# wallisc/TracerBoy

Measured on AMD Instinct MI355X. Metric: Msamples/s (WxHxspp/s), higher is better.
Workload: dtype f32; 1 GPU; cornell-box 1920x1080 64spp depth8; triangles=36, bvh_builder=sah, pipeline=lockstep, parallelism=tiles1, scene_in_lds=True, kernel_variant=matte

## Files before the change

include/tracerboy_hip.h:

```cpp
#ifndef TRACERBOY_HIP_H
#define TRACERBOY_HIP_H

#include <stdint.h>
#include "tb_abi.h"

#ifdef __cplusplus
extern "C" {
#endif

#define TB_OK 0
#define TB_E_INVALID -1
#define TB_E_NO_DEVICE -2
#define TB_E_IO -3
#define TB_E_PARSE -4
#define TB_E_DEVICE -5
#define TB_E_UNSUPPORTED -6
#define TB_E_NO_SCENE -7

typedef struct tb_context tb_context;

typedef struct tb_camera {
    float Position[3], LookAt[3], Right[3], Up[3];
    float LensHeight, FocalDistance;
} tb_camera;
// ... 135 lines not shown
typedef struct tb_launch_plan {
    int32_t pipeline;
    uint32_t groups;
    uint32_t high_occupancy_copy, full_variant;
    uint32_t stack_lds_entries, stack_overflow_entries;
    uint32_t compact_nodes;
    uint32_t prepass;
    uint32_t overlap_launches;
    uint32_t batch_frames, frame_group;
    uint32_t rule_pipeline, rule_copy, rule_prepass;
    uint32_t guided_groups;
    uint32_t costly_first;
} tb_launch_plan;
void tb_plan_defaults(tb_plan_input* in);
int tb_variant_waves_hi(const char* variant_name);
int tb_variant_stash_entries(const char* variant_name);
int tb_plan_launch(const tb_plan_input* in, tb_launch_plan* out);
uint32_t tb_frame_groups(uint32_t frames, uint32_t frame_group, uint32_t guided, uint32_t group, uint32_t* first_frame, uint32_t* num_frames);

int tb_host_scene_view(tb_context* ctx, TbSceneView* view);
int tb_make_frame_constants(tb_context* ctx, uint32_t width, uint32_t height, uint32_t frame,
                            const tb_output_settings* settings, float time_seed, TbPerFrameConstants* out);
float tb_last_render_ms(tb_context* ctx);
int tb_trace_closest(tb_context* ctx, uint32_t n, const float* origins, const float* dirs, float* out_t,
                     int32_t* out_material, float* out_bary, uint32_t* out_prim, uint32_t* out_geom,
                     float* out_normal, float* out_uv, uint32_t* out_boxes, uint32_t* out_tris);
int tb_device_math(tb_context* ctx, int fn, uint32_t n, const float* a, const float* b, float* out);

typedef struct tb_host_scene tb_host_scene;
int tb_host_scene_load(const char* pbrt_path, int bvh_builder, int load_flags, tb_host_scene** out, char* err, uint32_t err_len);
// ... 16 lines not shown
```

tracerboy_amd/api.py:

```python
import ctypes as C
import os

import numpy as np

from . import _ctypes_abi as abi

_HERE = os.path.dirname(os.path.abspath(__file__))
LIB_PATH = os.environ.get("TB_LIB", os.path.join(_HERE, "libtracerboy_hip.so"))

_lib = None


class TracerBoyError(RuntimeError):
    def __init__(self, code, message):
        super().__init__("tracerboy_hip error %d: %s" % (code, message))
        self.code = code


def lib():
    global _lib
    if _lib is not None:
        return _lib
    if not os.path.exists(LIB_PATH):
        raise ImportError("libtracerboy_hip.so is not built: run `python -m tracerboy_amd.build` "
# ... 29 lines not shown
        "tb_render_realtime": (C.c_int, [vp, C.c_uint32, C.c_uint32, P(abi.tb_output_settings), P(abi.tb_denoiser_settings), C.c_float]),
        "tb_read_realtime": (C.c_int, [vp, C.c_int, vp]),
        "tb_post_process": (C.c_int, [vp, P(abi.tb_post_settings), C.c_uint32, vp, vp]),
        "tb_read_averaged_luminance": (C.c_int, [vp, P(C.c_float)]),
        "tb_write_image_rgba8": (C.c_int, [C.c_char_p, C.c_uint32, C.c_uint32, vp]),
        "tb_write_image_f32": (C.c_int, [C.c_char_p, C.c_uint32, C.c_uint32, vp]),
        "tb_decode_image": (C.c_int, [C.c_char_p, P(C.c_uint32), P(C.c_uint32), P(C.c_int), P(C.c_int), vp]),
        "tb_read_aov": (C.c_int, [vp, C.c_int, vp]),
        "tb_accum_device_ptr": (C.c_int, [vp, P(vp), P(vp)]),
        "tb_read_stats": (C.c_int, [vp, P(abi.tb_readback_stats)]),
        "tb_read_wave_profile": (C.c_int, [vp, P(C.c_uint64)]),
        "tb_read_split_profile": (C.c_int, [vp, P(C.c_uint64)]),
        "tb_plan_defaults": (None, [P(abi.tb_plan_input)]),
        "tb_plan_launch": (C.c_int, [P(abi.tb_plan_input), P(abi.tb_launch_plan)]),
        "tb_variant_waves_hi": (C.c_int, [C.c_char_p]),
        "tb_invalidate_history": (None, [vp]),
        "tb_samples_rendered": (C.c_uint32, [vp]),
        "tb_select_pixel": (C.c_int, [vp, C.c_uint32, C.c_uint32]),
        "tb_set_tile_assignment": (C.c_int, [vp, C.c_uint32, C.c_uint32, C.c_uint32, C.c_uint32]),
        "tb_owned_pixels": (C.c_uint64, [vp, C.c_uint32, C.c_uint32]),
        "tb_pack_owned_device": (C.c_int, [vp, vp]),
        "tb_pack_owned_device_async": (C.c_int, [vp, vp]),
        "tb_stream": (vp, [vp]),
        "tb_unpack_gathered_device": (C.c_int, [vp, vp, vp, C.c_uint64, C.c_uint32, C.c_uint32, C.c_uint32, C.c_uint32, C.c_uint32, vp]),
        "tb_unpack_gathered_host": (C.c_int, [C.c_uint32, C.c_uint32, C.c_uint32, C.c_uint32, C.c_uint32, P(vp), vp]),
        "tb_set_option": (C.c_int, [vp, C.c_char_p, C.c_int64]),
        "tb_get_option": (C.c_int64, [vp, C.c_char_p]),
        "tb_host_scene_view": (C.c_int, [vp, P(abi.TbSceneView)]),
        "tb_make_frame_constants": (C.c_int, [vp, C.c_uint32, C.c_uint32, C.c_uint32, P(abi.tb_output_settings), C.c_float, P(abi.TbPerFrameConstants)]),
        "tb_last_render_ms": (C.c_float, [vp]),
# ... 31 lines not shown
    s = abi.tb_denoiser_settings()
    lib().tb_default_denoiser_settings(C.byref(s))
    return s


def GetDefaultPostProcessSettings():
    s = abi.tb_post_settings()
    lib().tb_default_post_settings(C.byref(s))
    return s


def VariantWavesHi(name):
    return int(lib().tb_variant_waves_hi(name.encode()))


def VariantStashEntries(name):
    return int(lib().tb_variant_stash_entries(name.encode()))


def PlanLaunch(**kw):
    pin = abi.tb_plan_input(); lib().tb_plan_defaults(C.byref(pin))
    for k, v in kw.items():
        if not hasattr(pin, k): raise KeyError(k)
        setattr(pin, k, v)
    plan = abi.tb_launch_plan()
    rc = lib().tb_plan_launch(C.byref(pin), C.byref(plan))
    if rc != 0: raise TracerBoyError(rc, "tb_plan_launch")
    return plan


# ... 306 lines not shown
```

tracerboy_amd/build.py:

```python
import concurrent.futures as cf
import hashlib
import os
import subprocess
import sys

ROOT = os.path.dirname(os.path.abspath(__file__))
REPO = os.path.dirname(ROOT)
CSRC = os.path.join(ROOT, "csrc")
OBJ = os.path.join(ROOT, "_build")
LIB = os.path.join(ROOT, "libtracerboy_hip.so")
CLI = os.path.join(ROOT, "tracerboy-hip")
HIPCC = os.environ.get("HIPCC", "/opt/rocm/bin/hipcc")
ARCH = os.environ.get("TB_ARCH", "gfx950")

COMMON = ["-O3", "-std=c++17", "-fPIC", "-ffp-contract=off", "-fno-fast-math", "-Wall", "-Wno-unused-function",
          "-Wno-unused-variable", "-Wno-unused-but-set-variable", "-I" + os.path.join(REPO, "include")] + os.environ.get("TB_EXTRA_FLAGS", "").split()
DEVICE = ["--offload-arch=" + ARCH, "-fno-slp-vectorize", "-mllvm", "-amdgpu-sched-strategy=max-ilp"]
SCHED_MEMORY_CLAUSE = ["-mllvm", "-amdgpu-sched-strategy=max-memory-clause"]
TU_SCHEDULER = {"kernels/pt_variant_vol4.hip": SCHED_MEMORY_CLAUSE, "kernels/pt_variant_surf.hip": SCHED_MEMORY_CLAUSE}


def device_flags(src):
    if src not in TU_SCHEDULER:
        return DEVICE
    base = [f for i, f in enumerate(DEVICE) if not f.startswith("-amdgpu-sched-strategy=")
            and not (f == "-mllvm" and i + 1 < len(DEVICE) and DEVICE[i + 1].startswith("-amdgpu-sched-strategy="))]
    return base + TU_SCHEDULER[src]

HOST_SRCS = ["host/pbrt_loader.cpp", "host/pbf_loader.cpp", "host/host_scene.cpp", "host/images.cpp", "host/image_decode.cpp", "host/image_formats.cpp", "host/bvh_build.cpp", "host/procedural.cpp", "host/context.cpp", "host/context_scene.cpp", "host/context_render.cpp", "host/pbrt_dump.cpp"]
KERNEL_SRCS = ["kernels/pt_kernels.hip", "kernels/post_kernels.hip", "kernels/bvh_kernels.hip", "kernels/rt_kernels.hip", "kernels/pt_variant_matte.hip", "kernels/pt_variant_matte5.hip", "kernels/pt_variant_env.hip", "kernels/pt_variant_env5.hip", "kernels/pt_variant_surf.hip",
               "kernels/pt_variant_sss.hip", "kernels/pt_variant_sss4.hip",
               "kernels/pt_variant_vol.hip", "kernels/pt_variant_vol4.hip", "kernels/pt_variant_full.hip",
               "kernels/pt_split_matte.hip", "kernels/pt_split_env.hip", "kernels/pt_split_surf.hip", "kernels/pt_split_sss.hip"]


def _deps_digest():
    h = hashlib.sha1()
    for base in (CSRC, os.path.join(REPO, "include")):
        for dp, _, fs in sorted(os.walk(base)):
            for f in sorted(fs):
                if f.endswith((".h", ".hpp", ".inc", ".cpp", ".hip")):
                    with open(os.path.join(dp, f), "rb") as fh:
                        h.update(f.encode()); h.update(fh.read())
    h.update(" ".join([f for f in COMMON + DEVICE if not f.startswith("-I")] + [k + " ".join(v) for k, v in sorted(TU_SCHEDULER.items())]).encode())
    return h.hexdigest()
# ... 55 lines not shown
```

tracerboy_amd/csrc/host/context.cpp:

```cpp
#include "context_internal.h"

using namespace tbhost;
using namespace tbctx;

namespace tbctx {

std::string g_createError;
std::atomic<int64_t> g_liveDeviceBytes{0};
#ifndef __HIP_DEVICE_COMPILE__
const Variant kVariants[] = {
    {0u, pt_launch_persistent_matte, "matte", pt_launch_persistent_matte5, TB_MATTE_WAVES, 0, wf_launch_matte, true, pt_launch_split_matte, 0u},
        {PT_FEAT_ENV, pt_launch_persistent_env, "env", pt_launch_persistent_env5, TB_ENV_WAVES, 1, wf_launch_env, true, pt_launch_split_env, TB_ENV_STASH},
    {PT_FEAT_ENV | PT_FEAT_SPECULAR | PT_FEAT_TEXTURES, pt_launch_persistent_surf, "surf", nullptr, 0, 2, wf_launch_surf, true, pt_launch_split_surf, 0u},
        {PT_FEAT_ENV | PT_FEAT_SPECULAR | PT_FEAT_TEXTURES | PT_FEAT_SSS, pt_launch_persistent_sss, "sss", pt_launch_persistent_sss4, TB_SSS_WAVES, 5,
            wf_launch_sss, false, pt_launch_split_sss, TB_SSS_STASH},
    {PT_FEAT_ENV | PT_FEAT_SPECULAR | PT_FEAT_TEXTURES | PT_FEAT_SSS | PT_FEAT_MIX, pt_launch_persistent_vol, "vol", pt_launch_persistent_vol4, TB_VOL_WAVES,
        3, wf_launch_vol, false, nullptr, TB_VOL_STASH},
        {PT_FEAT_ALL, pt_launch_persistent_full, "full", nullptr, 0, 4, nullptr, false, nullptr, 0u},
};
const int kNumVariants = (int)(sizeof(kVariants) / sizeof(kVariants[0]));
#endif

int fail(tb_context* c, int code, const std::string& msg) { if (c) c->err = msg; else g_createError = msg; return code; }

void ensure(DevBuf& b, size_t bytes)
{
// ... 176 lines not shown
}

int tb_material_count(tb_context* c) { return (c && c->hasScene) ? (int)c->scene.materials.size() : 0; }
int tb_get_material(tb_context* c, int id, TbMaterial* o)
{
    if (!c || !o) return TB_E_INVALID;
    if (!c->hasScene || id < 0 || id >= (int)c->scene.materials.size()) return fail(c, TB_E_INVALID, "material id out of range");
    *o = c->scene.materials[(size_t)id]; return TB_OK;
}
int tb_set_material(tb_context* c, int id, const TbMaterial* in)
{
    return guarded(c, [&]() {
        if (!in || !c->hasScene || id < 0 || id >= (int)c->scene.materials.size()) return fail(c, TB_E_INVALID, "material id out of range");
        c->scene.materials[(size_t)id] = *in;
        HIP_TRY(hipMemcpy((void*)&c->ds.materials[id].m, in, sizeof *in, hipMemcpyHostToDevice));
        if (c->sceneInLds) HIP_TRY(hipMemcpy((void*)(c->ds.ldsBlob + c->ds.offMaterials + sizeof(TbDevMaterial) * (size_t)id), in, sizeof *in,
            hipMemcpyHostToDevice));
        c->sceneFeatures = sceneFeatureMask(c->scene);
        c->ds.textureUse = sceneTextureUse(c);
        c->samplesRendered = 0;
        for (tb_context* p : c->peers) { const int rc = tb_set_material(p, id, in); if (rc != TB_OK) return rc; }
        return TB_OK;
    });
}

static int renderGroup(tb_context* c, uint32_t W, uint32_t H, uint32_t n, const tb_output_settings* s, float t)
{
    const uint32_t world = 1u + (uint32_t)c->peers.size();
    if (c->options.count("aov") && c->options["aov"]) return fail(c, TB_E_UNSUPPORTED, "tb_render: AOV targets are not gathered across the devices of a group");
    std::vector<tb_context*> all; all.push_back(c); for (tb_context* p : c->peers) all.push_back(p);
    for (uint32_t i = 0; i < world; i++) if (all[i]->tiles.world != world || all[i]->tiles.rank != i) { all[i]->tiles = TbTileMap{i, world, 64, 64};
        all[i]->samplesRendered = 0; }
// ... 285 lines not shown
    in->split_trav = 4; in->guided_groups = 1;
}
int tb_variant_stash_entries(const char* name)
{
    if (!name) return -1;
    for (int i = 0; i < tbctx::kNumVariants; i++) if (!strcmp(tbctx::kVariants[i].name, name)) return tbctx::kVariants[i].fnHi ? (int)tbctx::kVariants[i].stashHi : 0;
    return -1;
}
int tb_variant_waves_hi(const char* name)
{
    if (!name) return -1;
    for (int i = 0; i < tbctx::kNumVariants; i++) if (!strcmp(tbctx::kVariants[i].name,
        name)) return tbctx::kVariants[i].fnHi ? (int)tbctx::kVariants[i].wavesHi : 0;
    return -1;
}
uint32_t tb_frame_groups(uint32_t frames, uint32_t frameGroup, uint32_t guided, uint32_t group, uint32_t* firstFrame, uint32_t* numFrames)
{
    uint32_t lg = 0; while ((2u << lg) <= frameGroup) lg++;
    const uint32_t total = tb_fg_groups(frames, lg, guided ? 1u : 0u, 0xffffffffu, nullptr, nullptr);
    if (group < total) { uint32_t f0 = 0, l = 0; (void)tb_fg_groups(frames, lg, guided ? 1u : 0u, group, &f0, &l);
        if (firstFrame) *firstFrame = f0; if (numFrames) *numFrames = std::min(1u << l, frames - std::min(frames, f0)); }
    return total;
}

int tb_plan_launch(const tb_plan_input* in, tb_launch_plan* out)
{
    if (!in || !out || !in->width || !in->height) return TB_E_INVALID;
    PlanLaunch(*in, *out);
    return TB_OK;
}
// ... 111 lines not shown
    if (!strcmp(name, "overlap_trial_us_overlapped")) return (int64_t)(c->overlapTrial.best[0] * 1000.0f);
    if (!strcmp(name, "overlap_trial_us_one_at_a_time")) return (int64_t)(c->overlapTrial.best[1] * 1000.0f);
    if (!strcmp(name, "overlap_trial_phase")) return c->overlapTrial.phase;
    if (!strcmp(name, "last_plan_rule_pipeline")) return c->lastPlan.rule_pipeline;
    if (!strcmp(name, "last_plan_rule_copy")) return c->lastPlan.rule_copy;
    if (!strcmp(name, "last_plan_rule_prepass")) return c->lastPlan.rule_prepass;
    if (!strcmp(name, "last_plan_frame_group")) return c->lastPlan.frame_group;
    if (!strcmp(name, "last_plan_guided_groups")) return c->lastPlan.guided_groups;
    if (!strcmp(name, "last_plan_costly_first")) return c->lastPlan.costly_first;
    if (!strcmp(name, "debug_region_order_ptr")) return (int64_t)(uintptr_t)c->regionOrder[c->lastFgPar].p;
    if (!strcmp(name, "debug_region_cost_ptr")) return (int64_t)(uintptr_t)c->regionCost.p;
    if (!strcmp(name, "debug_live_device_bytes")) return g_liveDeviceBytes.load();
    if (!strcmp(name, "last_plan_stack_overflow")) return c->lastPlan.stack_overflow_entries;
    if (!strcmp(name, "last_split_waves")) return c->lastSplitWaves;
    if (!strcmp(name, "last_pipeline")) return c->lastPipeline;
    if (!strcmp(name, "last_variant")) { for (int i = 0; i < kNumVariants; i++) if (c->lastVariant == kVariants[i].name) return kVariants[i].id; return -1; }
    auto it = c->options.find(name); return it == c->options.end() ? 0 : it->second;
}

static void fillView(const HostScene& s, TbSceneView* v);
int tb_host_scene_view(tb_context* c, TbSceneView* v)
{
    if (!c || !v) return TB_E_INVALID;
    if (!c->hasScene) return fail(c, TB_E_NO_SCENE, "no scene loaded");
    fillView(c->scene, v);
    return TB_OK;
}

int tb_make_frame_constants(tb_context* c, uint32_t, uint32_t, uint32_t frame, const tb_output_settings* settings, float t, TbPerFrameConstants* out)
{
// ... 162 lines not shown
```

tracerboy_amd/csrc/host/context_internal.h:

```cpp
#pragma once
#include "host_scene.h"
#include "../kernels/pt_launch.h"
#include "../kernels/pt_device_features.h"
#include "launch_plan.h"

#include <hip/hip_runtime.h>

#include <algorithm>
#include <atomic>
#include <cstring>
#include <limits>
#include <cmath>
#include <map>
#include <stdexcept>
#include <string>
#include <vector>

using namespace tbhost;

extern "C" {
typedef hipError_t (*pt_variant_fn)(hipStream_t, const TbDeviceScene*, const TbPerFrameConstants*, const TbDeviceTargets*, uint32_t, uint32_t, uint32_t,
    uint32_t,
                                    const TbTileMap*, int, int, int);
hipError_t pt_launch_persistent_matte(hipStream_t, const TbDeviceScene*, const TbPerFrameConstants*, const TbDeviceTargets*, uint32_t, uint32_t, uint32_t,
    uint32_t, const TbTileMap*, int, int, int);
hipError_t pt_launch_persistent_env(hipStream_t, const TbDeviceScene*, const TbPerFrameConstants*, const TbDeviceTargets*, uint32_t, uint32_t, uint32_t,
    uint32_t, const TbTileMap*, int, int, int);
hipError_t pt_launch_persistent_surf(hipStream_t, const TbDeviceScene*, const TbPerFrameConstants*, const TbDeviceTargets*, uint32_t, uint32_t, uint32_t,
    uint32_t, const TbTileMap*, int, int, int);
hipError_t pt_launch_persistent_matte5(hipStream_t, const TbDeviceScene*, const TbPerFrameConstants*, const TbDeviceTargets*, uint32_t, uint32_t, uint32_t,
    uint32_t, const TbTileMap*, int, int, int);
hipError_t pt_launch_persistent_env5(hipStream_t, const TbDeviceScene*, const TbPerFrameConstants*, const TbDeviceTargets*, uint32_t, uint32_t, uint32_t,
    uint32_t, const TbTileMap*, int, int, int);
hipError_t pt_launch_persistent_sss(hipStream_t, const TbDeviceScene*, const TbPerFrameConstants*, const TbDeviceTargets*, uint32_t, uint32_t, uint32_t,
    uint32_t, const TbTileMap*, int, int, int);
hipError_t pt_launch_persistent_sss4(hipStream_t, const TbDeviceScene*, const TbPerFrameConstants*, const TbDeviceTargets*, uint32_t, uint32_t, uint32_t,
    uint32_t, const TbTileMap*, int, int, int);
hipError_t pt_launch_persistent_vol4(hipStream_t, const TbDeviceScene*, const TbPerFrameConstants*, const TbDeviceTargets*, uint32_t, uint32_t, uint32_t,
    uint32_t, const TbTileMap*, int, int, int);
hipError_t pt_launch_persistent_vol(hipStream_t, const TbDeviceScene*, const TbPerFrameConstants*, const TbDeviceTargets*, uint32_t, uint32_t, uint32_t,
    uint32_t, const TbTileMap*, int, int, int);
hipError_t pt_launch_persistent_full(hipStream_t, const TbDeviceScene*, const TbPerFrameConstants*, const TbDeviceTargets*, uint32_t, uint32_t, uint32_t,
    uint32_t, const TbTileMap*, int, int, int);
typedef hipError_t (*pt_split_fn)(hipStream_t, const TbDeviceScene*, const TbPerFrameConstants*, const TbDeviceTargets*, const TbSplitParams*, uint32_t,
    uint32_t, uint32_t, uint32_t,
// ... 20 lines not shown
hipError_t wf_launch_surf(hipStream_t, int, const TbDeviceScene*, const TbPerFrameConstants*, const WfParams*, const WfQueue*, const WfQueue*, const WfQueue*,
    const WfHits*, int, TbFloat4*, TbFloat4*, uint32_t);
hipError_t wf_launch_sss(hipStream_t, int, const TbDeviceScene*, const TbPerFrameConstants*, const WfParams*, const WfQueue*, const WfQueue*, const WfQueue*,
    const WfHits*, int, TbFloat4*, TbFloat4*, uint32_t);
hipError_t wf_launch_vol(hipStream_t, int, const TbDeviceScene*, const TbPerFrameConstants*, const WfParams*, const WfQueue*, const WfQueue*, const WfQueue*,
    const WfHits*, int, TbFloat4*, TbFloat4*, uint32_t);
}

namespace tbctx {
using namespace tbhost;

extern std::string g_createError;
#ifndef TB_MATTE_WAVES
#define TB_MATTE_WAVES 5
#endif
#ifndef TB_ENV_WAVES
#define TB_ENV_WAVES 6
#endif
#ifndef TB_SSS_WAVES
#define TB_SSS_WAVES 6
#endif
#ifndef TB_VOL_WAVES
#define TB_VOL_WAVES 4
#endif
#ifndef TB_ENV_STASH
#define TB_ENV_STASH 7
#endif
#ifndef TB_VOL_STASH
#define TB_VOL_STASH 0
#endif
#ifndef TB_SSS_STASH
#define TB_SSS_STASH 0
#endif
struct Variant { uint32_t features; pt_variant_fn fn; const char* name; pt_variant_fn fnHi; uint32_t wavesHi; int id; wf_variant_fn wf; bool pooled;
    pt_split_fn split; uint32_t stashHi; };
extern const Variant kVariants[];
extern const int kNumVariants;

extern std::atomic<int64_t> g_liveDeviceBytes;
struct DevBuf {
    void* p = nullptr; size_t bytes = 0;
    void release() { if (p) { (void)hipFree(p); g_liveDeviceBytes -= (int64_t)bytes; } p = nullptr; bytes = 0; }
};

}
using tbctx::DevBuf;

struct tb_context {
    int device = 0;
    hipStream_t stream = nullptr;
// ... 21 lines not shown
    DevBuf postOut, postRgba8, postHistogram, postAverage;
    DevBuf rtIndirect[2], rtMoment[2], rtFinal[2], rtDenoise[2], rtComposited;
    uint32_t rtActive = 0, rtWidth = 0, rtHeight = 0; int rtLast[5] = {-1, -1, -1, -1, -1};
    bool lastRenderRealtime = false; tb_camera prevCamera{};
    DevBuf wfCols[2][6], wfShadowCols[12], wfHitA, wfHitG, wfSamples, wfCounts, workCounter;
    uint64_t wfCapacity = 0, wfSampleCapacity = 0;
    int lastPipeline = 0;
    uint32_t samplesRendered = 0;
    tb_output_settings lastSettings{}; bool haveLastSettings = false;
    float lastTime = 0.0f;
    uint32_t selX = 0xffffffffu, selY = 0xffffffffu;
    TbTileMap tiles{0, 1, 64, 64};
    std::map<std::string, int64_t> options;
    float lastMs = 0.0f;
    std::string lastVariant;
    int lastNodeLayout = 0;
    int lastSlotLogCap = 0;
    struct PrepassTrial { uint64_t key = 0; int calls = 0, pending = 0, nWith = 0, nWithout = 0; float msWith = 0, msWithout = 0; bool keep = false;
        uint64_t stamp = 0; } prepassTrial;
    struct OverlapTrial { uint64_t key = 0; int phase = 0 ; int n[2] = {0, 0};
        float best[2] = {0, 0}; bool keep = true; } overlapTrial;
    struct CallRec { uint64_t key = 0; int mode = -1; bool deviceBound = false, settled = false, used = true; } callRec[8];
    hipEvent_t evCallEnd[8] = {nullptr, nullptr, nullptr, nullptr, nullptr, nullptr, nullptr, nullptr}; uint64_t callCount = 0; int lastOverlap = 0;
    tb_launch_plan lastPlan{};
    uint64_t kernelEventStamp = 0;
    uint32_t sceneGeneration = 0;
    float interiorWalkTriangleShare = 0;
    uint32_t hitPrimBits = 32, hitGeomBits = 32;
    int lastCompactHits = 0;
    DevBuf debugCounters;
// ... 64 lines not shown
```

tracerboy_amd/csrc/host/context_render.cpp:

```cpp
#include "context_internal.h"
#include "tb_vec.h"

namespace tbctx {

bool historyRelevantChange(const tb_output_settings& a, const tb_output_settings& b)
{
    return a.OutputType != b.OutputType || a.EnableNormalMaps != b.EnableNormalMaps || a.RenderModeRealTime != b.RenderModeRealTime ||
           a.DOFFocalDistance != b.DOFFocalDistance || a.ApertureWidth != b.ApertureWidth || a.FilterType != b.FilterType || a.FilterWidth != b.FilterWidth ||
           a.FireflyClampValue != b.FireflyClampValue || a.EnableNextEventEstimation != b.EnableNextEventEstimation ||
           a.EnableSamplingImportanceResampling != b.EnableSamplingImportanceResampling || a.EnableBlueNoise != b.EnableBlueNoise ||
               a.MaxBounces != b.MaxBounces ||
           a.DebugValue != b.DebugValue || a.DebugValue2 != b.DebugValue2;
}

void renderWavefront(tb_context* c, int variant, uint32_t W, uint32_t H, uint32_t firstFrame, uint32_t n, TbPerFrameConstants pf)
{
    auto opt = [&](const char* k, int64_t d) { auto it = c->options.find(k); return it == c->options.end() ? d : it->second; };
    const uint64_t pixels = (uint64_t)W * H;
    const uint64_t perFrame = (uint64_t)((W + 7) / 8) * ((H + 7) / 8) * 64;
    const uint64_t budget = (uint64_t)opt("wavefront_paths", 16ll << 20);
    const uint32_t segCap = (uint32_t)std::max<int64_t>(256, opt("wavefront_segment", 4096));
    uint32_t batch = (uint32_t)std::max<uint64_t>(1, std::min<uint64_t>(n, budget / perFrame));
    const uint64_t maxSegments = (perFrame * batch + segCap - 1) / segCap;
    const uint64_t capacity = maxSegments * segCap;
// ... 295 lines not shown
        pin.pipeline = 0; PlanLaunch(pin, plan); plan.rule_pipeline = TB_PLAN_RULE_SPLIT_NO_ROOM;
    }
    const bool wavefront = plan.pipeline == 2, pooled = plan.pipeline == 3, split = plan.pipeline == 4, groups = plan.groups != 0;
    const int64_t fg = opt("frame_group", 0);
    pt_variant_fn launch = plan.high_occupancy_copy ? v->fnHi : v->fn;
    size_t overflowHalf = 0;
    TbDeviceScene dsLaunch = c->ds; dsLaunch.stackOverflow = nullptr; dsLaunch.stackOverflowLanes = 0;
    if (plan.stack_overflow_entries) {
        const int numCUs = deviceCUs(c);
        const uint32_t lanes = 2u * 8u * (uint32_t)numCUs * 256u;
        ensure(c->stackOverflow, (size_t)plan.stack_overflow_entries * lanes * 4 * 2);
        overflowHalf = (size_t)plan.stack_overflow_entries * lanes;
        dsLaunch.stackDepth = plan.stack_lds_entries; dsLaunch.stackOverflow = (uint32_t*)c->stackOverflow.p; dsLaunch.stackOverflowLanes = lanes;
    }
    if (plan.full_variant && v != &kVariants[kNumVariants - 1]) { v = &kVariants[kNumVariants - 1]; launch = v->fn; c->lastVariant = v->name; }
    if (opt("node_layout", 0) == 1 && !twoLevel && !c->sceneInLds && !c->ds.nodesC && !c->compactTried) {
        ensureCompactNodes(c); dsLaunch.nodesC = c->ds.nodesC; dsLaunch.quant = c->ds.quant;
        pin.has_compact_nodes = c->ds.nodesC ? 1u : 0u; PlanLaunch(pin, plan);
    }
    const bool compactNodes = plan.compact_nodes != 0;
    if (!compactNodes) dsLaunch.nodesC = nullptr;
    c->lastNodeLayout = compactNodes ? 1 : 0;
    bool prepass = plan.prepass == TB_PLAN_PREPASS_ON;
    if (plan.prepass == TB_PLAN_PREPASS_TRIAL) {
        tb_context::PrepassTrial& t = c->prepassTrial;
        const uint64_t key = ((uint64_t)W << 48) ^ ((uint64_t)H << 32) ^ ((uint64_t)n << 12) ^ ((uint64_t)s.MaxBounces << 4) ^ ((uint64_t)c->sceneGeneration <<
            24) ^ (uint64_t)(uintptr_t)launch;
        if (t.key != key) { t = tb_context::PrepassTrial(); t.key = key; }
        if (t.pending) {
            float ms = 0;
// ... 90 lines not shown
                    HIP_TRY(hipMemsetAsync(c->fgSamples[par].p, 0, pixels * batch * 16, overlap ? c->side[par] : c->stream));
                }
            auto warmFrameGroupForm = [&](uint32_t par, bool withHits) {
                TbDeviceTargets warm = tg; warm.samples = (TbFloat4*)c->fgSamples[par].p; warm.workCounter = (uint32_t*)c->workCounter.p + par * 128u;
                const int numCUs = deviceCUs(c);
                if (c->fgSlotLog[par].bytes < 16ull * numCUs * 16 * 8) ensure(c->fgSlotLog[par], 16ull * numCUs * 16 * 8);
                warm.slotLog = (unsigned long long*)c->fgSlotLog[par].p; warm.slotLogCap = 16; warm.launchEpoch = ++c->launchEpoch;
                warm.primaryHits = withHits ? (unsigned long long*)c->fgHits[par].p : nullptr; warm.firstBounce = withHits && firstBounce ? 1u : 0u;
                warm.hitStamp = withHits ? hitStampOf(warm.launchEpoch) : 0u; warm.hitPrimBits = hitPrimBits; warm.hitGeomBits = c->hitGeomBits;
                TbDeviceScene dsPar = dsLaunch; if (dsPar.stackOverflow) dsPar.stackOverflow += par * overflowHalf;
                hipStream_t st = overlap ? c->side[par] : c->stream;
                HIP_TRY(launch(st, &dsPar, &pf, &warm, W, H, c->samplesRendered, 0, &c->tiles, withHits ? 0 : (c->sceneInLds ? 1 : 0), 0, 0));
                HIP_TRY(hipStreamSynchronize(st));
            };
            if (overlap && std::find(c->warmedLaunchers.begin(), c->warmedLaunchers.end(), (const void*)launch) == c->warmedLaunchers.end()) {
                if (twoLevel) { for (uint32_t par = 0; par < 2; par++) warmFrameGroupForm(par, false); }
                else {
                    TbDeviceTargets none = tg; none.samples = nullptr;
                    TbDeviceScene dsWarm = c->ds; dsWarm.nodesC = nullptr;
                    for (uint32_t par = 0; par < 2; par++)
                        HIP_TRY(launch(c->side[par], &dsWarm, &pf, &none, W, H, c->samplesRendered, 0, &c->tiles, c->sceneInLds ? 1 : 0, 0, 0));
                }
                c->warmedLaunchers.push_back((const void*)launch);
            }
            if (prepass) {
                for (uint32_t par = 0; par < 2u; par++)
                    if (c->fgHits[par].bytes < pixels * batch * hitRecordBytes) {
                        HIP_TRY(hipStreamSynchronize(c->side[par])); HIP_TRY(hipStreamSynchronize(c->stream));
                        ensure(c->fgHits[par], pixels * batch * hitRecordBytes);
                        HIP_TRY(hipMemsetAsync(c->fgHits[par].p, 0, pixels * batch * hitRecordBytes, overlap ? c->side[par] : c->stream));
                    }
// ... 61 lines not shown
```

tracerboy_amd/csrc/host/context_scene.cpp:

```cpp
#include "context_internal.h"

namespace tbctx {

void releaseScene(tb_context* c)
{
    for (DevBuf& b : c->sceneBufs) b.release();
    c->sceneBufs.clear();
    memset(&c->ds, 0, sizeof c->ds);
}

uint32_t sceneFeatureMask(const HostScene& s)
{
    uint32_t f = 0;
    if (!s.envMap.empty()) f |= PT_FEAT_ENV;
    for (const TbMaterial& m : s.materials) {
        if ((m.Flags & TB_MAT_NO_SPECULAR) == 0 && (m.Flags & TB_MAT_MIX) == 0) f |= PT_FEAT_SPECULAR;
        if (m.albedoIndex != TB_INVALID_TEXTURE || m.emissiveIndex != TB_INVALID_TEXTURE || m.specularMapIndex != TB_INVALID_TEXTURE ||
            m.normalMapIndex != TB_INVALID_TEXTURE) f |= PT_FEAT_TEXTURES | PT_FEAT_SPECULAR;
        if (m.Flags & TB_MAT_SUBSURFACE_SCATTER) f |= PT_FEAT_SSS;
        if (m.Flags & TB_MAT_MIX) f |= PT_FEAT_MIX;
    }
    for (const TbLight& l : s.lights) if (l.LightType != TB_LIGHT_TYPE_AREA) f |= PT_FEAT_EXT;
    return f;
}
// ... 306 lines not shown
        }
        {
            std::vector<TbTriB> perm(s.trisB.size() * TB_LDS_TRI_COPIES);
            for (size_t i = 0; i < s.trisB.size(); i++)
                for (int kz = 0; kz < 3; kz++)
                    for (int sw = 0; sw < 2; sw++) {
                        int kx = kz == 2 ? 0 : kz + 1, ky = kx == 2 ? 0 : kx + 1;
                        if (sw) std::swap(kx, ky);
                        const TbTriB& t = s.trisB[i]; TbTriB q = t;
                        const float* src[3] = {t.v0, t.v1, t.v2}; float* dst[3] = {q.v0, q.v1, q.v2};
                        for (int v = 0; v < 3; v++) { dst[v][0] = src[v][kx]; dst[v][1] = src[v][ky]; dst[v][2] = src[v][kz]; }
                        perm[i * TB_LDS_TRI_COPIES + (size_t)(kz * 2 + sw)] = q;
                    }
            d.offTris = put(perm.data(), perm.size() * sizeof(TbTriB));
        }
        d.offHitGroups = put(devHit.data(), devHit.size() * sizeof(TbDevHitGroup));
        d.offIndices = put(s.indexBuffer.data(), s.indexBuffer.size() * 4);
        d.offVertices = put(s.vertexBuffer.data(), s.vertexBuffer.size() * 4);
        d.offMaterials = put(devMat.data(), devMat.size() * sizeof(TbDevMaterial));
        d.offLights = put(devLight.data(), devLight.size() * sizeof(TbDevLight));
        while (blob.size() % 16) blob.push_back(0);
        size_t budget = (size_t)opt("lds_scene_budget", 40 * 1024);
        c->sceneInLds = blob.size() + (size_t)d.stackDepth * 256 * 4 <= budget && opt("scene_in_lds", 1) != 0 && !twoLevel;
        if (c->sceneInLds) { d.ldsBlob = upload(c, blob); d.ldsBlobBytes = (uint32_t)blob.size(); }
        else { d.ldsBlob = nullptr; d.ldsBlobBytes = 0; }
        d.parkMin = (uint32_t)std::max<int64_t>(1, opt("park_min", c->sceneInLds ? 2 : 24));
    }
    HIP_TRY(hipStreamSynchronize(c->stream));
    c->sceneFeatures = sceneFeatureMask(s);
    c->hasScene = true;
    c->samplesRendered = 0;
}

}
```

tracerboy_amd/csrc/host/launch_plan.h:

```cpp
#pragma once
#include <stdint.h>
#include <algorithm>
#include "../../../include/tracerboy_hip.h"
#include "../kernels/pt_scene.h"

namespace tbhost {

inline void PlanLaunch(const tb_plan_input& in, tb_launch_plan& p)
{
    p = tb_launch_plan{};
    const bool plain = !in.count_rays && !in.aov && !in.realtime && !in.selected_pixel;
    const int64_t pipe = in.pipeline == 4 ? 0 : in.pipeline;
    p.pipeline = (int32_t)pipe;
    if (in.pipeline == 4 && in.variant_has_split && plain && !in.two_level) {
        const uint64_t trav = (uint64_t)std::max<int64_t>(1, in.split_trav),
            shade = in.split_shade > 0 ? (uint64_t)in.split_shade : (in.scene_in_lds ? 4u : 6u);
        uint64_t ring = 256; while (ring < 256u * shade) ring *= 2;
        const uint64_t entries = (in.split_stack_cap > 0 && (uint64_t)in.split_stack_cap < in.stack_depth && !in.scene_in_lds) ? (uint64_t)in.split_stack_cap :
            in.stack_depth;
        const uint64_t lds = entries * trav * 256u + (in.scene_in_lds ? ((uint64_t)in.lds_blob_bytes + 15u) / 16u * 16u : 0u) + shade * 128u * 48u + ring *
            4u + 16u;
        const bool fits = lds <= 160u * 1024u && 4ull * std::max<uint64_t>(1, in.owned_regions) <= 0xfffffull && (trav + shade) * 64u <= 1024u;
        if (fits) { p.pipeline = 4; p.rule_pipeline = TB_PLAN_RULE_SPLIT; return; }
        p.rule_pipeline = TB_PLAN_RULE_SPLIT_NO_ROOM;
// ... 72 lines not shown
```

tracerboy_amd/csrc/kernels/pt_common.hpp:

```cpp
#pragma once
#include <hip/hip_runtime.h>
#include "pt_device.hpp"

namespace {
using namespace pt;

constexpr int BLOCK = 256;

template <bool SCENE_LDS>
__device__ __forceinline__ void make_refs(SceneRefs& sc, const TbDeviceScene& ds, const uint8_t* blob)
{
    if (SCENE_LDS) {
        sc.nodes = blob + ds.offNodes; sc.tris = (const TbTriB*)__builtin_assume_aligned(blob + ds.offTris, 16); sc.trisPermuted = 1;
        sc.hitGroups = (const TbDevHitGroup*)(blob + ds.offHitGroups); sc.indices = (const uint32_t*)(blob + ds.offIndices);
        sc.vertices = (const float*)(blob + ds.offVertices); sc.materials = (const TbDevMaterial*)(blob + ds.offMaterials);
        sc.lights = (const TbDevLight*)(blob + ds.offLights);
    } else {
        sc.nodes = (const uint8_t*)ds.nodes; sc.tris = ds.tris; sc.trisPermuted = 0; sc.hitGroups = ds.hitGroups; sc.indices = ds.indexBuffer;
            sc.vertices = ds.vertexBuffer;
        sc.materials = ds.materials; sc.lights = ds.lights;
    }
    sc.numHitGroups = ds.numHitGroups; sc.numIndices = ds.numIndices; sc.numVertexFloats = ds.numVertexFloats;
    sc.numMaterials = ds.numMaterials; sc.numLights = ds.numLights;
}

__device__ __forceinline__ bool block_region(const TbTileMap& tiles, uint32_t W, uint32_t H, uint32_t region, uint32_t& bx, uint32_t& by)
{
    if (tiles.world <= 1) { const uint32_t blocksX = (W + 15u) / 16u; bx = region % blocksX; by = region / blocksX; return true; }
    const uint32_t subX = tiles.tileW / 16u, perTile = subX * (tiles.tileH / 16u);
    const uint32_t k = region / perTile, sub = region % perTile;
    const uint32_t tilesX = (W + tiles.tileW - 1) / tiles.tileW, t = tiles.rank + k * tiles.world;
    bx = (t % tilesX) * subX + sub % subX; by = (t / tilesX) * (tiles.tileH / 16u) + sub / subX;
    return true;
}

__device__ __noinline__ uint32_t claim_work_item(uint32_t* counters, uint32_t regions, uint32_t numGroups, uint32_t banded, const uint32_t* order = nullptr)
// ... 67 lines not shown
```

tracerboy_amd/csrc/kernels/pt_scene.h:

```cpp
#pragma once
#include "../../../include/tb_abi.h"
#include <stdint.h>

#define TB_LDS_NODE_STRIDE 80u
#define TB_DEVICE_REF_MASK 0x7fffffffu
#define TB_LDS_TRI_COPIES 6u

struct __attribute__((aligned(16))) TbDevHitGroup { uint32_t MaterialIndex, vFirst, iFirst, pad; };
struct __attribute__((aligned(16))) TbDevMaterial { TbMaterial m; uint32_t pad[3]; };
struct __attribute__((aligned(16))) TbDevLight { TbLight l; uint32_t pad[2]; };

struct TbDeviceScene {
    const TbNodeB* nodes;
    const TbTriB* tris;
    const TbNodeC* nodesC;
    TbQuantFrame quant;
    uint32_t rootRef;
    const TbInstanceB* instances; uint32_t numInstances;
    uint32_t numNodes, numTris;
    float rootCenter[3], rootHalf[3];
    const TbDevHitGroup* hitGroups;      uint32_t numHitGroups;
    const uint32_t* indexBuffer;         uint32_t numIndices;
    const float* vertexBuffer;           uint32_t numVertexFloats;
    const TbDevMaterial* materials;      uint32_t numMaterials;
    const TbTextureData* textureData;    uint32_t numTextureData;
    const TbDevLight* lights;            uint32_t numLights;
    const TbImageDesc* images;           uint32_t numImages;
    const TbFloat4* texelPool;
    const TbFloat4* envMap;              uint32_t envWidth, envHeight;
    const TbFloat4* blueNoise0;
    const TbFloat4* blueNoise1;
    TbConfigConstants config;
    uint32_t alphaTest;
    uint32_t textureUse;
    uint32_t parkMin;
    uint32_t stackDepth;
    uint32_t* stackOverflow;     uint32_t stackOverflowLanes;
    const uint8_t* ldsBlob;      uint32_t ldsBlobBytes;
    uint32_t offNodes, offTris, offHitGroups, offIndices, offVertices, offMaterials, offLights;
};

#ifndef TB_COSTLY_STEP
#define TB_COSTLY_STEP 8
#endif
struct TbDeviceTargets {
    TbFloat4* output;
    TbFloat4* jittered;
    TbFloat4* aovNormals;
    TbFloat4* aovWorldPos0, *aovWorldPos1;
    TbFloat4* aovCustom;
    float* aovDepth;
    TbFloat4* aovEmissive;
    uint32_t* stats;
    unsigned long long* rayStats;
// ... 66 lines not shown
```

tracerboy_amd/csrc/kernels/pt_variant.inc:

```
#include <hip/hip_runtime.h>
#include "pt_common.hpp"
#include "pt_launch.h"

namespace {
#include "pt_persistent.inc"
#ifndef PT_ONLY_PERSISTENT
#include "pt_stream.inc"
#endif
}

#define PT_CAT2(a, b) a##b
#define PT_CAT(a, b) PT_CAT2(a, b)

extern "C" hipError_t PT_CAT(pt_launch_persistent_, PT_NAME)(hipStream_t stream, const TbDeviceScene* ds, const TbPerFrameConstants* pf,
    const TbDeviceTargets* tg,
                                                            uint32_t W, uint32_t H, uint32_t firstFrame, uint32_t numFrames, const TbTileMap* tiles,
                                                            int sceneInLds, int countRays, int pipeline)
{
    uint32_t blocks = tb_persistent_grid(W, H, *tiles);
    if (blocks == 0) return hipSuccess;
    size_t lds = (size_t)ds->stackDepth * BLOCK * 4 + (sceneInLds ? ds->ldsBlobBytes : 0);
#ifdef PT_LDS_STASH
    if (!sceneInLds && tg->samples && !ds->numInstances) lds += (size_t)PT_LDS_STASH * BLOCK * 4;
#endif
// ... 15 lines not shown
            uint32_t lgG = 0; while ((2u << lgG) <= tg->frameGroup) lgG++; \
            const uint64_t items = (uint64_t)blocks * tb_fg_groups(numFrames, lgG, guidedLaunch ? 1u : 0u, 0xffffffffu, nullptr, nullptr), \
                resident = (uint64_t)(perCU > 0 ? perCU : 1) * numCUs; \
            grid.x = (uint32_t)(items < 2 * resident ? items : 2 * resident);  \
            if (grid.x == 0) grid.x = 1;  \
            if (!tg->slotLog || !tg->slotLogCap || grid.x > 16u * (uint32_t)numCUs) return hipErrorInvalidValue; \
            e = hipMemsetAsync(tg->slotLog, 0, (size_t)grid.x * tg->slotLogCap * 8, stream); if (e != hipSuccess) return e; \
            e = hipMemsetAsync(tg->workCounter, 0, 512, stream); if (e != hipSuccess) return e; } \
        hipLaunchKernelGGL((__VA_ARGS__), grid, block, lds, stream, *ds, *pf, *tg, W, H, firstFrame, numFrames, *tiles); } while (0)
#ifndef PT_ONLY_PERSISTENT
#define PT_PICK(L, C) do { if (pipeline == 1) PT_LAUNCH(pt_stream<PT_FEATURES, L, C>); else PT_LAUNCH(pt_persistent<PT_FEATURES, L, C, false>); } while (0)
#else
#define PT_PICK(L, C) do { if (pipeline != 0) return hipErrorInvalidValue; PT_LAUNCH(pt_persistent<PT_FEATURES, L, C, false>); } while (0)
#endif
    if (tg->samples && (countRays || pipeline != 0)) return hipErrorInvalidValue;
#if PT_COUNT
    if (countRays) { if (sceneInLds) PT_PICK(true, true); else PT_PICK(false, true); return hipGetLastError(); }
#else
    if (countRays) return hipErrorInvalidValue;
#endif
#ifdef PT_ONLY_PERSISTENT
    if (ds->numInstances) {
        if (!tg->samples || sceneInLds || ds->nodesC) return hipErrorInvalidValue;
        if (ds->stackOverflow) {
            if (ds->stackOverflowLanes < 2u * 8u * (uint32_t)numCUs * BLOCK) return hipErrorInvalidValue;
            PT_LAUNCH(pt_persistent<PT_FEATURES, false, false, true, true, false, true>);
        } else PT_LAUNCH(pt_persistent<PT_FEATURES, false, false, true, false, false, true>);
        return hipGetLastError();
    }
#elif !(PT_FEATURES & PT_FEAT_EXT)
// ... 61 lines not shown
        if (ds->stackOverflowLanes < 2u * 8u * (uint32_t)numCUs * BLOCK) return hipErrorInvalidValue;
        if (sceneInLds) PT_LAUNCH(pt_persistent<PT_FEATURES, true, false, true, true>); else PT_LAUNCH(pt_persistent<PT_FEATURES, false, false, true, true>);
        return hipGetLastError();
    }
#endif
    if (ds->stackOverflow) return hipErrorInvalidValue;
#ifdef TB_EXP_PROFILE_GROUPS
    if (tg->samples) { if (sceneInLds) PT_LAUNCH(pt_persistent<PT_FEATURES, true, true, true>);
        else PT_LAUNCH(pt_persistent<PT_FEATURES, false, true, true>); }
#else
    if (tg->samples) { if (guidedLaunch) PT_LAUNCH(pt_persistent<PT_FEATURES, true, false, true, false, false, false, false, false, true>);
        else if (sceneInLds) PT_LAUNCH(pt_persistent<PT_FEATURES, true, false, true>);
        else PT_LAUNCH(pt_persistent<PT_FEATURES, false, false, true>); }
#endif
    else if (sceneInLds) PT_PICK(true, false); else PT_PICK(false, false);
#undef PT_PICK
#undef PT_LAUNCH
    return hipGetLastError();
}

#if !(PT_FEATURES & PT_FEAT_EXT) && !defined(PT_ONLY_PERSISTENT)
#include "wf_types.h"
#define PT_HAS_POOLED (!(PT_FEATURES & (PT_FEAT_SSS | PT_FEAT_MIX)))
namespace {
#include "wf_kernels.inc"
#if PT_HAS_POOLED
#include "pt_pooled.inc"
#endif
}
extern "C" hipError_t PT_CAT(wf_launch_, PT_NAME)(hipStream_t stream, int stage, const TbDeviceScene* ds, const TbPerFrameConstants* pf, const WfParams* wp,
// ... 65 lines not shown
```

Measured before the change: 7170 Msamples/s.

## Keep only BVH in LDS and add a six-wave matte LDS kernel copy

```diff
diff --git a/include/tracerboy_hip.h b/include/tracerboy_hip.h
--- a/include/tracerboy_hip.h
+++ b/include/tracerboy_hip.h
@@ -173,6 +173,7 @@
 } tb_launch_plan;
 void tb_plan_defaults(tb_plan_input* in);
 int tb_variant_waves_hi(const char* variant_name);
+int tb_variant_waves_lds(const char* variant_name);
 int tb_variant_stash_entries(const char* variant_name);
 int tb_plan_launch(const tb_plan_input* in, tb_launch_plan* out);
 uint32_t tb_frame_groups(uint32_t frames, uint32_t frame_group, uint32_t guided, uint32_t group, uint32_t* first_frame, uint32_t* num_frames);
diff --git a/tracerboy_amd/api.py b/tracerboy_amd/api.py
--- a/tracerboy_amd/api.py
+++ b/tracerboy_amd/api.py
@@ -67,6 +67,7 @@
         "tb_plan_defaults": (None, [P(abi.tb_plan_input)]),
         "tb_plan_launch": (C.c_int, [P(abi.tb_plan_input), P(abi.tb_launch_plan)]),
         "tb_variant_waves_hi": (C.c_int, [C.c_char_p]),
+        "tb_variant_waves_lds": (C.c_int, [C.c_char_p]),
         "tb_invalidate_history": (None, [vp]),
         "tb_samples_rendered": (C.c_uint32, [vp]),
         "tb_select_pixel": (C.c_int, [vp, C.c_uint32, C.c_uint32]),
@@ -128,6 +129,10 @@
     return int(lib().tb_variant_waves_hi(name.encode()))
 
 
+def VariantWavesLds(name):
+    return int(lib().tb_variant_waves_lds(name.encode()))
+
+
 def VariantStashEntries(name):
     return int(lib().tb_variant_stash_entries(name.encode()))
 
diff --git a/tracerboy_amd/build.py b/tracerboy_amd/build.py
--- a/tracerboy_amd/build.py
+++ b/tracerboy_amd/build.py
@@ -17,7 +17,8 @@
           "-Wno-unused-variable", "-Wno-unused-but-set-variable", "-I" + os.path.join(REPO, "include")] + os.environ.get("TB_EXTRA_FLAGS", "").split()
 DEVICE = ["--offload-arch=" + ARCH, "-fno-slp-vectorize", "-mllvm", "-amdgpu-sched-strategy=max-ilp"]
 SCHED_MEMORY_CLAUSE = ["-mllvm", "-amdgpu-sched-strategy=max-memory-clause"]
-TU_SCHEDULER = {"kernels/pt_variant_vol4.hip": SCHED_MEMORY_CLAUSE, "kernels/pt_variant_surf.hip": SCHED_MEMORY_CLAUSE}
+SCHED_DEFAULT = []
+TU_SCHEDULER = {"kernels/pt_variant_vol4.hip": SCHED_MEMORY_CLAUSE, "kernels/pt_variant_surf.hip": SCHED_MEMORY_CLAUSE, "kernels/pt_variant_matte6.hip": SCHED_DEFAULT}
 
 
 def device_flags(src):
@@ -28,7 +29,7 @@
     return base + TU_SCHEDULER[src]
 
 HOST_SRCS = ["host/pbrt_loader.cpp", "host/pbf_loader.cpp", "host/host_scene.cpp", "host/images.cpp", "host/image_decode.cpp", "host/image_formats.cpp", "host/bvh_build.cpp", "host/procedural.cpp", "host/context.cpp", "host/context_scene.cpp", "host/context_render.cpp", "host/pbrt_dump.cpp"]
-KERNEL_SRCS = ["kernels/pt_kernels.hip", "kernels/post_kernels.hip", "kernels/bvh_kernels.hip", "kernels/rt_kernels.hip", "kernels/pt_variant_matte.hip", "kernels/pt_variant_matte5.hip", "kernels/pt_variant_env.hip", "kernels/pt_variant_env5.hip", "kernels/pt_variant_surf.hip",
+KERNEL_SRCS = ["kernels/pt_kernels.hip", "kernels/post_kernels.hip", "kernels/bvh_kernels.hip", "kernels/rt_kernels.hip", "kernels/pt_variant_matte.hip", "kernels/pt_variant_matte5.hip", "kernels/pt_variant_matte6.hip", "kernels/pt_variant_env.hip", "kernels/pt_variant_env5.hip", "kernels/pt_variant_surf.hip",
                "kernels/pt_variant_sss.hip", "kernels/pt_variant_sss4.hip",
                "kernels/pt_variant_vol.hip", "kernels/pt_variant_vol4.hip", "kernels/pt_variant_full.hip",
                "kernels/pt_split_matte.hip", "kernels/pt_split_env.hip", "kernels/pt_split_surf.hip", "kernels/pt_split_sss.hip"]
diff --git a/tracerboy_amd/csrc/host/context.cpp b/tracerboy_amd/csrc/host/context.cpp
--- a/tracerboy_amd/csrc/host/context.cpp
+++ b/tracerboy_amd/csrc/host/context.cpp
@@ -9,7 +9,8 @@
 std::atomic<int64_t> g_liveDeviceBytes{0};
 #ifndef __HIP_DEVICE_COMPILE__
 const Variant kVariants[] = {
-    {0u, pt_launch_persistent_matte, "matte", pt_launch_persistent_matte5, TB_MATTE_WAVES, 0, wf_launch_matte, true, pt_launch_split_matte, 0u},
+    {0u, pt_launch_persistent_matte, "matte", pt_launch_persistent_matte5, TB_MATTE_WAVES, 0, wf_launch_matte, true, pt_launch_split_matte, 0u,
+        pt_launch_persistent_matte6, TB_MATTE_LDS_WAVES},
         {PT_FEAT_ENV, pt_launch_persistent_env, "env", pt_launch_persistent_env5, TB_ENV_WAVES, 1, wf_launch_env, true, pt_launch_split_env, TB_ENV_STASH},
     {PT_FEAT_ENV | PT_FEAT_SPECULAR | PT_FEAT_TEXTURES, pt_launch_persistent_surf, "surf", nullptr, 0, 2, wf_launch_surf, true, pt_launch_split_surf, 0u},
         {PT_FEAT_ENV | PT_FEAT_SPECULAR | PT_FEAT_TEXTURES | PT_FEAT_SSS, pt_launch_persistent_sss, "sss", pt_launch_persistent_sss4, TB_SSS_WAVES, 5,
@@ -216,8 +217,6 @@
         if (!in || !c->hasScene || id < 0 || id >= (int)c->scene.materials.size()) return fail(c, TB_E_INVALID, "material id out of range");
         c->scene.materials[(size_t)id] = *in;
         HIP_TRY(hipMemcpy((void*)&c->ds.materials[id].m, in, sizeof *in, hipMemcpyHostToDevice));
-        if (c->sceneInLds) HIP_TRY(hipMemcpy((void*)(c->ds.ldsBlob + c->ds.offMaterials + sizeof(TbDevMaterial) * (size_t)id), in, sizeof *in,
-            hipMemcpyHostToDevice));
         c->sceneFeatures = sceneFeatureMask(c->scene);
         c->ds.textureUse = sceneTextureUse(c);
         c->samplesRendered = 0;
@@ -533,6 +532,12 @@
         name)) return tbctx::kVariants[i].fnHi ? (int)tbctx::kVariants[i].wavesHi : 0;
     return -1;
 }
+int tb_variant_waves_lds(const char* name)
+{
+    if (!name) return -1;
+    for (int i = 0; i < tbctx::kNumVariants; i++) if (!strcmp(tbctx::kVariants[i].name, name)) return tbctx::kVariants[i].fnLds ? (int)tbctx::kVariants[i].wavesLds : 0;
+    return -1;
+}
 uint32_t tb_frame_groups(uint32_t frames, uint32_t frameGroup, uint32_t guided, uint32_t group, uint32_t* firstFrame, uint32_t* numFrames)
 {
     uint32_t lg = 0; while ((2u << lg) <= frameGroup) lg++;
@@ -674,6 +679,7 @@
     if (!strcmp(name, "last_plan_stack_overflow")) return c->lastPlan.stack_overflow_entries;
     if (!strcmp(name, "last_split_waves")) return c->lastSplitWaves;
     if (!strcmp(name, "last_pipeline")) return c->lastPipeline;
+    if (!strcmp(name, "last_copy_waves")) return c->lastCopyWaves;
     if (!strcmp(name, "last_variant")) { for (int i = 0; i < kNumVariants; i++) if (c->lastVariant == kVariants[i].name) return kVariants[i].id; return -1; }
     auto it = c->options.find(name); return it == c->options.end() ? 0 : it->second;
 }
diff --git a/tracerboy_amd/csrc/host/context_internal.h b/tracerboy_amd/csrc/host/context_internal.h
--- a/tracerboy_amd/csrc/host/context_internal.h
+++ b/tracerboy_amd/csrc/host/context_internal.h
@@ -29,6 +29,8 @@
 hipError_t pt_launch_persistent_surf(hipStream_t, const TbDeviceScene*, const TbPerFrameConstants*, const TbDeviceTargets*, uint32_t, uint32_t, uint32_t,
     uint32_t, const TbTileMap*, int, int, int);
 hipError_t pt_launch_persistent_matte5(hipStream_t, const TbDeviceScene*, const TbPerFrameConstants*, const TbDeviceTargets*, uint32_t, uint32_t, uint32_t,
+    uint32_t, const TbTileMap*, int, int, int);
+hipError_t pt_launch_persistent_matte6(hipStream_t, const TbDeviceScene*, const TbPerFrameConstants*, const TbDeviceTargets*, uint32_t, uint32_t, uint32_t,
     uint32_t, const TbTileMap*, int, int, int);
 hipError_t pt_launch_persistent_env5(hipStream_t, const TbDeviceScene*, const TbPerFrameConstants*, const TbDeviceTargets*, uint32_t, uint32_t, uint32_t,
     uint32_t, const TbTileMap*, int, int, int);
@@ -79,6 +81,9 @@
 #ifndef TB_MATTE_WAVES
 #define TB_MATTE_WAVES 5
 #endif
+#ifndef TB_MATTE_LDS_WAVES
+#define TB_MATTE_LDS_WAVES 6
+#endif
 #ifndef TB_ENV_WAVES
 #define TB_ENV_WAVES 6
 #endif
@@ -98,7 +103,7 @@
 #define TB_SSS_STASH 0
 #endif
 struct Variant { uint32_t features; pt_variant_fn fn; const char* name; pt_variant_fn fnHi; uint32_t wavesHi; int id; wf_variant_fn wf; bool pooled;
-    pt_split_fn split; uint32_t stashHi; };
+    pt_split_fn split; uint32_t stashHi; pt_variant_fn fnLds; uint32_t wavesLds; };
 extern const Variant kVariants[];
 extern const int kNumVariants;
 
@@ -150,6 +155,7 @@
     std::map<std::string, int64_t> options;
     float lastMs = 0.0f;
     std::string lastVariant;
+    uint32_t lastCopyWaves = 0;
     int lastNodeLayout = 0;
     int lastSlotLogCap = 0;
     struct PrepassTrial { uint64_t key = 0; int calls = 0, pending = 0, nWith = 0, nWithout = 0; float msWith = 0, msWithout = 0; bool keep = false;
diff --git a/tracerboy_amd/csrc/host/context_render.cpp b/tracerboy_amd/csrc/host/context_render.cpp
--- a/tracerboy_amd/csrc/host/context_render.cpp
+++ b/tracerboy_amd/csrc/host/context_render.cpp
@@ -333,6 +333,9 @@
         dsLaunch.stackDepth = plan.stack_lds_entries; dsLaunch.stackOverflow = (uint32_t*)c->stackOverflow.p; dsLaunch.stackOverflowLanes = lanes;
     }
     if (plan.full_variant && v != &kVariants[kNumVariants - 1]) { v = &kVariants[kNumVariants - 1]; launch = v->fn; c->lastVariant = v->name; }
+    c->lastCopyWaves = launch == v->fnHi ? v->wavesHi : 0u;
+    if (launch == v->fnHi && v->fnLds && groups && c->sceneInLds && !twoLevel && !count && !plan.stack_overflow_entries && !plan.prepass &&
+        LdsCopyFits(v->wavesLds, c->ds.stackDepth, c->ds.ldsBlobBytes)) { launch = v->fnLds; c->lastCopyWaves = v->wavesLds; }
     if (opt("node_layout", 0) == 1 && !twoLevel && !c->sceneInLds && !c->ds.nodesC && !c->compactTried) {
         ensureCompactNodes(c); dsLaunch.nodesC = c->ds.nodesC; dsLaunch.quant = c->ds.quant;
         pin.has_compact_nodes = c->ds.nodesC ? 1u : 0u; PlanLaunch(pin, plan);
@@ -453,7 +456,7 @@
                 HIP_TRY(hipStreamSynchronize(st));
             };
             if (overlap && std::find(c->warmedLaunchers.begin(), c->warmedLaunchers.end(), (const void*)launch) == c->warmedLaunchers.end()) {
-                if (twoLevel) { for (uint32_t par = 0; par < 2; par++) warmFrameGroupForm(par, false); }
+                if (twoLevel || launch == v->fnLds) { for (uint32_t par = 0; par < 2; par++) warmFrameGroupForm(par, false); }
                 else {
                     TbDeviceTargets none = tg; none.samples = nullptr;
                     TbDeviceScene dsWarm = c->ds; dsWarm.nodesC = nullptr;
diff --git a/tracerboy_amd/csrc/host/context_scene.cpp b/tracerboy_amd/csrc/host/context_scene.cpp
--- a/tracerboy_amd/csrc/host/context_scene.cpp
+++ b/tracerboy_amd/csrc/host/context_scene.cpp
@@ -344,14 +344,12 @@
                     }
             d.offTris = put(perm.data(), perm.size() * sizeof(TbTriB));
         }
-        d.offHitGroups = put(devHit.data(), devHit.size() * sizeof(TbDevHitGroup));
-        d.offIndices = put(s.indexBuffer.data(), s.indexBuffer.size() * 4);
-        d.offVertices = put(s.vertexBuffer.data(), s.vertexBuffer.size() * 4);
-        d.offMaterials = put(devMat.data(), devMat.size() * sizeof(TbDevMaterial));
-        d.offLights = put(devLight.data(), devLight.size() * sizeof(TbDevLight));
         while (blob.size() % 16) blob.push_back(0);
+        auto r16 = [](size_t b) { return (b + 15) / 16 * 16; };
+        const size_t shadingBytes = r16(devHit.size() * sizeof(TbDevHitGroup)) + r16(s.indexBuffer.size() * 4) + r16(s.vertexBuffer.size() * 4) +
+            r16(devMat.size() * sizeof(TbDevMaterial)) + r16(devLight.size() * sizeof(TbDevLight));
         size_t budget = (size_t)opt("lds_scene_budget", 40 * 1024);
-        c->sceneInLds = blob.size() + (size_t)d.stackDepth * 256 * 4 <= budget && opt("scene_in_lds", 1) != 0 && !twoLevel;
+        c->sceneInLds = blob.size() + shadingBytes + (size_t)d.stackDepth * 256 * 4 <= budget && opt("scene_in_lds", 1) != 0 && !twoLevel;
         if (c->sceneInLds) { d.ldsBlob = upload(c, blob); d.ldsBlobBytes = (uint32_t)blob.size(); }
         else { d.ldsBlob = nullptr; d.ldsBlobBytes = 0; }
         d.parkMin = (uint32_t)std::max<int64_t>(1, opt("park_min", c->sceneInLds ? 2 : 24));
diff --git a/tracerboy_amd/csrc/host/launch_plan.h b/tracerboy_amd/csrc/host/launch_plan.h
--- a/tracerboy_amd/csrc/host/launch_plan.h
+++ b/tracerboy_amd/csrc/host/launch_plan.h
@@ -5,6 +5,13 @@
 #include "../kernels/pt_scene.h"
 
 namespace tbhost {
+
+inline bool LdsCopyFits(uint32_t waves, uint32_t stackDepth, uint32_t ldsBlobBytes)
+{
+    if (!waves) return false;
+    const uint64_t share = (160u * 1024u / waves) / 512u * 512u, need = ((uint64_t)stackDepth * 1024u + ldsBlobBytes + 128u + 511u) / 512u * 512u;
+    return need <= share;
+}
 
 inline void PlanLaunch(const tb_plan_input& in, tb_launch_plan& p)
 {
diff --git a/tracerboy_amd/csrc/kernels/pt_common.hpp b/tracerboy_amd/csrc/kernels/pt_common.hpp
--- a/tracerboy_amd/csrc/kernels/pt_common.hpp
+++ b/tracerboy_amd/csrc/kernels/pt_common.hpp
@@ -10,16 +10,9 @@
 template <bool SCENE_LDS>
 __device__ __forceinline__ void make_refs(SceneRefs& sc, const TbDeviceScene& ds, const uint8_t* blob)
 {
-    if (SCENE_LDS) {
-        sc.nodes = blob + ds.offNodes; sc.tris = (const TbTriB*)__builtin_assume_aligned(blob + ds.offTris, 16); sc.trisPermuted = 1;
-        sc.hitGroups = (const TbDevHitGroup*)(blob + ds.offHitGroups); sc.indices = (const uint32_t*)(blob + ds.offIndices);
-        sc.vertices = (const float*)(blob + ds.offVertices); sc.materials = (const TbDevMaterial*)(blob + ds.offMaterials);
-        sc.lights = (const TbDevLight*)(blob + ds.offLights);
-    } else {
-        sc.nodes = (const uint8_t*)ds.nodes; sc.tris = ds.tris; sc.trisPermuted = 0; sc.hitGroups = ds.hitGroups; sc.indices = ds.indexBuffer;
-            sc.vertices = ds.vertexBuffer;
-        sc.materials = ds.materials; sc.lights = ds.lights;
-    }
+    if (SCENE_LDS) { sc.nodes = blob + ds.offNodes; sc.tris = (const TbTriB*)__builtin_assume_aligned(blob + ds.offTris, 16); sc.trisPermuted = 1; }
+    else { sc.nodes = (const uint8_t*)ds.nodes; sc.tris = ds.tris; sc.trisPermuted = 0; }
+    sc.hitGroups = ds.hitGroups; sc.indices = ds.indexBuffer; sc.vertices = ds.vertexBuffer; sc.materials = ds.materials; sc.lights = ds.lights;
     sc.numHitGroups = ds.numHitGroups; sc.numIndices = ds.numIndices; sc.numVertexFloats = ds.numVertexFloats;
     sc.numMaterials = ds.numMaterials; sc.numLights = ds.numLights;
 }
diff --git a/tracerboy_amd/csrc/kernels/pt_scene.h b/tracerboy_amd/csrc/kernels/pt_scene.h
--- a/tracerboy_amd/csrc/kernels/pt_scene.h
+++ b/tracerboy_amd/csrc/kernels/pt_scene.h
@@ -37,7 +37,7 @@
     uint32_t stackDepth;
     uint32_t* stackOverflow;     uint32_t stackOverflowLanes;
     const uint8_t* ldsBlob;      uint32_t ldsBlobBytes;
-    uint32_t offNodes, offTris, offHitGroups, offIndices, offVertices, offMaterials, offLights;
+    uint32_t offNodes, offTris;
 };
 
 #ifndef TB_COSTLY_STEP
diff --git a/tracerboy_amd/csrc/kernels/pt_variant.inc b/tracerboy_amd/csrc/kernels/pt_variant.inc
--- a/tracerboy_amd/csrc/kernels/pt_variant.inc
+++ b/tracerboy_amd/csrc/kernels/pt_variant.inc
@@ -53,6 +53,11 @@
 #define PT_PICK(L, C) do { if (pipeline != 0) return hipErrorInvalidValue; PT_LAUNCH(pt_persistent<PT_FEATURES, L, C, false>); } while (0)
 #endif
     if (tg->samples && (countRays || pipeline != 0)) return hipErrorInvalidValue;
+#ifdef PT_ONLY_LDS_GROUPS
+    if (!tg->samples || !sceneInLds || countRays || ds->numInstances || tg->primaryHits || ds->nodesC || ds->stackOverflow) return hipErrorInvalidValue;
+    if (guidedLaunch) PT_LAUNCH(pt_persistent<PT_FEATURES, true, false, true, false, false, false, false, false, true>);
+    else PT_LAUNCH(pt_persistent<PT_FEATURES, true, false, true>);
+#else
 #if PT_COUNT
     if (countRays) { if (sceneInLds) PT_PICK(true, true); else PT_PICK(false, true); return hipGetLastError(); }
 #else
@@ -144,6 +149,7 @@
         else PT_LAUNCH(pt_persistent<PT_FEATURES, false, false, true>); }
 #endif
     else if (sceneInLds) PT_PICK(true, false); else PT_PICK(false, false);
+#endif
 #undef PT_PICK
 #undef PT_LAUNCH
     return hipGetLastError();
diff --git a/tracerboy_amd/csrc/kernels/pt_variant_matte6.hip b/tracerboy_amd/csrc/kernels/pt_variant_matte6.hip
--- /dev/null
+++ b/tracerboy_amd/csrc/kernels/pt_variant_matte6.hip
@@ -0,0 +1,11 @@
+#include "pt_device_features.h"
+#define PT_FEATURES 0u
+#define PT_NAME matte6
+#define PT_COUNT 0
+#define PT_ONLY_PERSISTENT 1
+#define PT_ONLY_LDS_GROUPS 1
+#ifndef TB_MATTE_LDS_WAVES
+#define TB_MATTE_LDS_WAVES 6
+#endif
+#define PT_PERSISTENT_ATTR __attribute__((amdgpu_waves_per_eu(TB_MATTE_LDS_WAVES)))
+#include "pt_variant.inc"
```

Result: faster. 7469 Msamples/s, median of 6 (+4.2%).
